# cornell-c2s2/dsp

Measured on AMD Instinct MI355X. Metric: MFCC frames/sec (512-pt FFT, 40 mel, 13 coeffs), higher is better.
Workload: dtype f32

## Files before the change

dsp_amd/csrc/mfcc_device.hpp:

```cpp
#pragma once

#include <hip/hip_runtime.h>

#include <type_traits>

#include "mfcc_kernels.hpp"

namespace dsp {

namespace {

struct c32 { float x, y; };
typedef float f2v __attribute__((ext_vector_type(2)));
typedef int i2v __attribute__((ext_vector_type(2)));
typedef float f4v __attribute__((ext_vector_type(4)));

__device__ __forceinline__ c32 cadd(c32 a, c32 b) { return {a.x + b.x, a.y + b.y}; }
__device__ __forceinline__ c32 csub(c32 a, c32 b) { return {a.x - b.x, a.y - b.y}; }
__device__ __forceinline__ c32 cmul(c32 a, c32 w) { return {a.x * w.x - a.y * w.y, a.x * w.y + a.y * w.x}; }
__device__ __forceinline__ c32 cmul_mi(c32 a) { return {a.y, -a.x}; }

__device__ __forceinline__ void radix4(c32 (&s)[4])
{
    const c32 t0 = cadd(s[0], s[2]), t1 = csub(s[0], s[2]);
    const c32 t2 = cadd(s[1], s[3]), t3 = cmul_mi(csub(s[1], s[3]));
    s[0] = cadd(t0, t2);
    s[1] = cadd(t1, t3);
    s[2] = csub(t0, t2);
    s[3] = csub(t1, t3);
}

__device__ __forceinline__ void wave_lds_sync()
{
    __builtin_amdgcn_fence(__ATOMIC_RELEASE, "wavefront");
    __builtin_amdgcn_wave_barrier();
    __builtin_amdgcn_fence(__ATOMIC_ACQUIRE, "wavefront");
}

__device__ __forceinline__ void swap_hi32(float &a, float &b)
{
    auto r = __builtin_amdgcn_permlane32_swap(__float_as_uint(a), __float_as_uint(b), false, false);
    a = __uint_as_float(r[0]);
    b = __uint_as_float(r[1]);
}
__device__ __forceinline__ void swap_odd16(float &a, float &b)
{
    auto r = __builtin_amdgcn_permlane16_swap(__float_as_uint(a), __float_as_uint(b), false, false);
    a = __uint_as_float(r[0]);
    b = __uint_as_float(r[1]);
}

template <int CTRL>
__device__ __forceinline__ float dpp(float v)
{
    return __int_as_float(__builtin_amdgcn_update_dpp(0, __float_as_int(v), CTRL, 0xF, 0xF, true));
}
constexpr int DPP_QUAD_1032 = 0xB1;
constexpr int DPP_QUAD_2301 = 0x4E;
constexpr int DPP_ROW_HALF_MIRROR = 0x141;
constexpr int DPP_ROW_MIRROR = 0x140;

template <int CTRL>
__device__ __forceinline__ unsigned dppu(unsigned v)
{
    return (unsigned)__builtin_amdgcn_update_dpp(0, (int)v, CTRL, 0xF, 0xF, true);
}
__device__ __forceinline__ float wave_max_nonneg(float f)
{
    unsigned v = __float_as_uint(f);
    v = max(v, dppu<DPP_QUAD_1032>(v));
    v = max(v, dppu<DPP_QUAD_2301>(v));
    v = max(v, dppu<DPP_ROW_HALF_MIRROR>(v));
    v = max(v, dppu<DPP_ROW_MIRROR>(v));
    const unsigned r0 = __builtin_amdgcn_readlane(v, 0), r1 = __builtin_amdgcn_readlane(v, 16);
    const unsigned r2 = __builtin_amdgcn_readlane(v, 32), r3 = __builtin_amdgcn_readlane(v, 48);
    return __uint_as_float(max(max(r0, r1), max(r2, r3)));
}

constexpr int LDS_XCHG = 0;
constexpr int LDS_PART = 2048 + 64;
constexpr int LDS_LOGMEL = LDS_PART + 320;
constexpr int LDS_WAVE_BYTES = LDS_LOGMEL + 320;
constexpr int LDS_TILE_BYTES = 64 * 16 * 4;
constexpr int LDS_POOL_BYTES = 32 * 16;
constexpr int LDS_STOP_BYTES = 64 * kStopFusedUnits * 8;
static_assert(LDS_WAVE_BYTES % 16 == 0, "keep the carve 16-byte aligned");
struct FrameCursor {
    long f, chunk_end, chunk_first, stride, n;
    long clip;
    long jump_clips;
    int t, t0, fpc, chunk, jump_t;
    long clip0;
    __device__ __forceinline__ void init(long wave, long n_waves, int chunk_, long n_, int fpc_)
    {
        chunk = chunk_; n = n_; fpc = fpc_;
        stride = n_waves * chunk;
        chunk_first = wave * chunk;
        f = chunk_first;
        chunk_end = f + chunk < n ? f + chunk : n;
        clip0 = 0; t0 = 0; jump_clips = 0; jump_t = 0;
        if (fpc > 0) {
            clip0 = f / fpc; t0 = (int)(f - clip0 * fpc);
            jump_clips = stride / fpc; jump_t = (int)(stride - jump_clips * fpc);
        }
        clip = clip0; t = t0;
    }
    __device__ __forceinline__ bool valid() const { return f < n; }
    __device__ __forceinline__ void next(int step)
    {
        f += step;
        if (f >= chunk_end) {
            chunk_first += stride;
            f = chunk_first;
            chunk_end = f + chunk < n ? f + chunk : n;
            clip0 += jump_clips; t0 += jump_t;
            if (t0 >= fpc) { t0 -= fpc; ++clip0; }
            clip = clip0; t = t0;
        } else if (fpc > 0) {
            t += step;
            while (t >= fpc) { t -= fpc; ++clip; }
        }
    }
};

template <bool CLIPS>
struct WaveCursor {
    long f, off;
    long clip;
    long chunk_f, chunk_off;
    long chunk_clip;
    long stride_f, stride_off;
    long clip_off, clip_stride;
    long jump_clips;
    int remaining;
    int left, chunk;
    int t, t0, fpc, jump_t, hop;
    __device__ __forceinline__ void init(long wave, long n_waves, int chunk_, long n, int fpc_, int hop_, long clip_stride_)
    {
        chunk = chunk_; fpc = fpc_; hop = hop_; clip_stride = clip_stride_;
        stride_f = n_waves * chunk;
        chunk_f = wave * chunk;
        f = chunk_f;
        left = chunk - 1;
        const long n_chunks = (n + chunk - 1) / chunk;
        const long mine = wave < n_chunks ? (n_chunks - 1 - wave) / n_waves + 1 : 0;
        const bool owns_last = mine > 0 && (n_chunks - 1 - wave) % n_waves == 0;
        remaining = (int)(mine * chunk - (owns_last ? n_chunks * chunk - n : 0));
        clip = chunk_clip = 0; t = t0 = 0; jump_t = 0; jump_clips = 0; clip_off = 0;
        if (CLIPS) {
            chunk_clip = f / fpc; t0 = (int)(f - chunk_clip * fpc);
            jump_clips = stride_f / fpc; jump_t = (int)(stride_f - jump_clips * fpc);
            stride_off = jump_clips * clip_stride;
            chunk_off = chunk_clip * clip_stride;
            clip = chunk_clip; t = t0; clip_off = chunk_off;
            off = clip_off + (long)t * hop;
        } else {
            stride_off = stride_f * hop;
            chunk_off = chunk_f * hop;
            off = chunk_off;
        }
    }
    __device__ __forceinline__ bool valid() const { return remaining > 0; }
    __device__ __forceinline__ void next()
    {
        --remaining;
        const bool in_chunk = left > 0;
        left = in_chunk ? left - 1 : chunk - 1;
        chunk_f += in_chunk ? 0 : stride_f;
        f = in_chunk ? f + 1 : chunk_f;
        if (CLIPS) {
            const bool wrap = t + 1 == fpc;
            const int t_in = wrap ? 0 : t + 1;
            const long clip_in = clip + (wrap ? 1 : 0);
            const long clip_off_in = clip_off + (wrap ? clip_stride : 0);
            const long off_in = wrap ? clip_off_in : off + hop;
            const int t0_raw = t0 + (in_chunk ? 0 : jump_t);
            const bool carry = t0_raw >= fpc;
            t0 = carry ? t0_raw - fpc : t0_raw;
            chunk_clip += in_chunk ? 0 : jump_clips + (carry ? 1 : 0);
            chunk_off += in_chunk ? 0 : stride_off + (carry ? clip_stride : 0);
            t = in_chunk ? t_in : t0;
            clip = in_chunk ? clip_in : chunk_clip;
            clip_off = in_chunk ? clip_off_in : chunk_off;
            off = in_chunk ? off_in : chunk_off + t0 * hop;
        } else {
            chunk_off += in_chunk ? 0 : stride_off;
            off = in_chunk ? off + hop : chunk_off;
        }
    }
};

struct RaggedCursor {
    long f, off, clip;
    const ClipSpan *spans;
    const int *chunk_span;
    int chunk_k, n_waves;
    int remaining;
    int left, chunk;
    int t, clip_left;
    int hop, n_samples;
    __device__ __forceinline__ void enter(const ClipSpan &s)
    {
        t = (int)(f - s.frame0);
        off = s.off + (long)t * hop;
        clip_left = s.frames - 1 - t;
        n_samples = s.n;
    }
    __device__ __forceinline__ void init(long wave, long n_waves_, int chunk_, long n, int hop_, const ClipSpan *spans_, long n_spans)
    {
        chunk = chunk_; hop = hop_; n_waves = (int)n_waves_; spans = spans_;
        chunk_span = reinterpret_cast<const int *>(spans_ + n_spans);
        chunk_k = (int)wave;
        left = chunk - 1;
        const long n_chunks = (n + chunk - 1) / chunk;
        const long mine = wave < n_chunks ? (n_chunks - 1 - wave) / n_waves_ + 1 : 0;
        const bool owns_last = mine > 0 && (n_chunks - 1 - wave) % n_waves_ == 0;
        remaining = (int)(mine * chunk - (owns_last ? n_chunks * chunk - n : 0));
        f = (long)chunk_k * chunk; off = 0; clip = 0; t = 0; clip_left = 0; n_samples = 0;
        if (remaining > 0) { clip = chunk_span[chunk_k]; enter(spans[clip]); }
    }
    __device__ __forceinline__ bool valid() const { return remaining > 0; }
    __device__ __forceinline__ void next()
    {
        if (--remaining <= 0) return;
        if (left > 0 && clip_left > 0) {
            --left; ++f; --clip_left; ++t; off += hop;
            return;
        }
        if (left > 0) { --left; ++f; ++clip; }
        else {
            left = chunk - 1;
            chunk_k += n_waves;
            f = (long)chunk_k * chunk;
            clip = chunk_span[chunk_k];
        }
        enter(spans[clip]);
    }
};

struct ClipCursor {
    long f, off, clip;
    long n_clips, n_waves, clip_stride;
    const ClipSpan *spans;
    int left, remaining, t, hop, fpc, n_samples;
    __device__ __forceinline__ void enter()
    {
        t = 0;
        if (clip >= n_clips) { remaining = 0; return; }
        remaining = 2;
        if (spans) {
            const ClipSpan s = spans[clip];
            off = s.off; n_samples = s.n; left = s.frames - 1;
        } else {
            off = clip * clip_stride; left = fpc - 1;
        }
    }
    __device__ __forceinline__ void init(long wave, long n_waves_, long n_clips_, int fpc_, int hop_, long clip_stride_, const ClipSpan *spans_,
                                         int samples_per_clip)
    {
        n_clips = n_clips_; n_waves = n_waves_; clip_stride = clip_stride_; spans = spans_; hop = hop_; fpc = fpc_; n_samples = samples_per_clip;
        f = 0; off = 0; left = 0; clip = wave;
        enter();
    }
    __device__ __forceinline__ bool valid() const { return remaining > 0; }
    __device__ __forceinline__ void next()
    {
        ++f;
        if (left > 0) { --left; ++t; off += hop; }
        else { clip += n_waves; enter(); }
    }
};

__device__ __forceinline__ const Mfcc512Args *kernarg_of_mfcc512()
{
#if defined(__HIP_DEVICE_COMPILE__)
    return (const Mfcc512Args *)__builtin_amdgcn_kernarg_segment_ptr();
#else
    return nullptr;
#endif
}

}

}
```

dsp_amd/csrc/mfcc_kernels.hip:

```cpp
#include "diag_guard.hpp"
#include <hip/hip_runtime.h>

#include <algorithm>

#include "mfcc_device.hpp"

#ifndef DSP_DIAG_MODE
#define DSP_DIAG_MODE 0
#endif
#ifndef DSP_PREFETCH
#define DSP_PREFETCH 2
#endif
#ifndef DSP_PRIO_LOAD
#define DSP_PRIO_LOAD 0
#endif
#ifndef DSP_PRIO_FFT
#define DSP_PRIO_FFT 0
#endif
#ifndef DSP_PRIO_FFT2
#define DSP_PRIO_FFT2 1
#endif
#ifndef DSP_PRIO_UNT
#define DSP_PRIO_UNT 2
#endif
#ifndef DSP_PRIO_MEL
#define DSP_PRIO_MEL 3
#endif
#ifndef DSP_PRIO_TILE
#define DSP_PRIO_TILE 3
#endif
#define DSP_SETPRIO(from, to) do { if ((from) != (to)) __builtin_amdgcn_s_setprio(to); } while (0)

namespace dsp {

#ifdef DSP_PF_STAMPS
__device__ unsigned long long g_pf_stamps[8 * 1024];
#define PF_STAMP(k) do { if ((threadIdx.x & 63) == 0 && blockIdx.x < 256) g_pf_stamps[(blockIdx.x * 4 + (threadIdx.x >> 6)) * 8 + (k)] = __builtin_amdgcn_s_memtime(); } while (0)
hipError_t read_pf_stamps(unsigned long long *host, int count) { return hipMemcpyFromSymbol(host, HIP_SYMBOL(g_pf_stamps), sizeof(unsigned long long) * (size_t)count); }
#else
#define PF_STAMP(k) do { } while (0)
#endif

namespace {

template <typename V>
__device__ __forceinline__ V ld_frame(const V *p, bool stream) { return stream ? __builtin_nontemporal_load(p) : *p; }

template <int FLEN, int IN, bool STREAM>
__device__ __forceinline__ void load_frame(const void *__restrict__ base, long off, int lane, int frame_len, c32 (&z)[4])
{
#pragma unroll
    for (int a = 0; a < 4; ++a) {
        const int i = 2 * (lane + 64 * a);
        const int flen = FLEN ? FLEN : frame_len;
        const bool both = i + 1 < flen, one = i < flen;
        if (IN == 0) {
            const float *src = static_cast<const float *>(base) + off;
            if (both) {
                const f2v v = ld_frame(reinterpret_cast<const f2v *>(src + i), STREAM);
                z[a] = {v.x, v.y};
            } else if (one) {
                z[a] = {src[i], 0.0f};
            } else {
                z[a] = {0.0f, 0.0f};
            }
        } else if (IN == 1) {
            const short *src = static_cast<const short *>(base) + off;
            int v = 0;
            if (both) v = ld_frame(reinterpret_cast<const int *>(src + i), STREAM);
            else if (one) v = (int)(unsigned short)src[i];
            z[a] = {__int_as_float(v), 0.0f};
        } else {
            const short *src = static_cast<const short *>(base) + 2 * off;
            i2v v = {0, 0};
            if (both) v = ld_frame(reinterpret_cast<const i2v *>(src + 2 * i), STREAM);
            else if (one) v.x = *reinterpret_cast<const int *>(src + 2 * i);
            z[a] = {__int_as_float(v.x), __int_as_float(v.y)};
        }
    }
}

template <int IN>
__device__ __forceinline__ c32 unpack_pcm16(c32 raw)
{
    const int a = __float_as_int(raw.x), b = __float_as_int(raw.y);
    if (IN == 1) return {(float)(short)(a & 0xFFFF), (float)(a >> 16)};
    if (IN == 2) return {(float)(short)(a & 0xFFFF), (float)(short)(b & 0xFFFF)};
    return {(float)((short)(a & 0xFFFF) + (a >> 16)), (float)((short)(b & 0xFFFF) + (b >> 16))};
}

}

template <int DCT_SPLIT, int DCT_LEN, int GATHER, int FLEN, int IN, int TILE, bool CLIPS, int POOL = 0, bool RAGGED = false>
#ifndef DSP_WAVES_PER_EU
#define DSP_WAVES_PER_EU 4
#endif
__global__ __launch_bounds__(256) __attribute__((amdgpu_waves_per_eu(DSP_WAVES_PER_EU))) void mfcc512_wave_kernel(const Mfcc512Args args)
{
    static_assert(!POOL || (TILE && CLIPS), "pooling lives in the tile epilogue of the clip-mode kernel");
    static_assert(!RAGGED || (CLIPS && !POOL), "ragged batches: clip mode, coefficients stored");
    constexpr int KS = DCT_SPLIT == 2 ? DCT_LEN / 2 : DCT_LEN;
    constexpr int CT = DCT_SPLIT == 2 ? 2 : 1;
    constexpr int WAVE_BYTES = LDS_WAVE_BYTES + (TILE ? LDS_TILE_BYTES : 0) + (POOL == 1 ? LDS_POOL_BYTES : (POOL == 2 ? LDS_STOP_BYTES : 0));
    extern __shared__ __attribute__((aligned(16))) char smem[];
    const int lane = threadIdx.x & 63;
    const int wib = __builtin_amdgcn_readfirstlane(threadIdx.x >> 6);
    char *wl = smem + wib * WAVE_BYTES;
    float *etile = reinterpret_cast<float *>(wl + LDS_WAVE_BYTES);
    double *pool_acc = reinterpret_cast<double *>(wl + LDS_WAVE_BYTES + LDS_TILE_BYTES);
    (void)etile; (void)pool_acc;
    float2 *xchg = reinterpret_cast<float2 *>(wl + LDS_XCHG);
    float *pbuf = reinterpret_cast<float *>(wl + LDS_XCHG);
    float *part = reinterpret_cast<float *>(wl + LDS_PART);
    float *lmel = reinterpret_cast<float *>(wl + LDS_LOGMEL);

    const LaneTables512 *__restrict__ T = args.tables;

    float win[8];
    constexpr float in_scale = IN == 0 ? 1.0f : (IN == 3 ? 1.0f / 65536.0f : 1.0f / 32768.0f);
#pragma unroll
    for (int i = 0; i < 8; ++i) win[i] = T->win[i][lane] * in_scale;
    c32 tw1[3], tw2[3], tw3[3], twp[2];
#pragma unroll
    for (int q = 0; q < 3; ++q) {
        tw1[q] = {T->tw1[2 * q][lane], T->tw1[2 * q + 1][lane]};
        tw2[q] = {T->tw2[2 * q][lane], T->tw2[2 * q + 1][lane]};
        tw3[q] = {T->tw3[2 * q][lane], T->tw3[2 * q + 1][lane]};
    }
    twp[0] = {T->twp[0][lane], T->twp[1][lane]};
    twp[1] = {T->twp[2][lane], T->twp[3][lane]};
    float melw[kMelChunk];
#pragma unroll
    for (int i = 0; i < kMelChunk; ++i) melw[i] = T->mel_w[i][lane];
    const int mel_k0 = T->mel_k0[lane];
    int gat[GATHER];
#pragma unroll
    for (int g = 0; g < GATHER; ++g) gat[g] = T->mel_src[g][lane];
    float dctw[(DCT_LEN + 3) & ~3];
    constexpr bool A_IN_REGS = CT * KS <= 10 && !POOL;
    float dcta[CT][KS];
    float *a_lds = reinterpret_cast<float *>(smem + 4 * WAVE_BYTES);
    (void)a_lds;
    if (TILE && !A_IN_REGS) {
        for (int i = threadIdx.x; i < CT * KS * 64; i += 256) a_lds[i] = (&T->dct_a[0][0][0])[(i / (KS * 64)) * (kDctSteps * 64) + i % (KS * 64)];
        __syncthreads();
    }
    if (TILE && A_IN_REGS) {
#pragma unroll
        for (int ct = 0; ct < CT; ++ct)
#pragma unroll
            for (int s = 0; s < KS; ++s) dcta[ct][s] = T->dct_a[ct][s][lane];
    } else if (!TILE) {
#pragma unroll
        for (int i = 0; i < DCT_LEN; ++i) dctw[i] = T->dct_w[i][lane];
    }
    const int n_mels = args.n_mels, n_mfcc = args.n_mfcc;
    constexpr int DCT_STRIDE = (DCT_LEN + 3) & ~3;
    const int dct_rd = (lane % DCT_SPLIT) * DCT_STRIDE;
    const int lmel_wr = (lane / DCT_LEN) * DCT_STRIDE + lane % DCT_LEN;
    const int dct_c = lane / DCT_SPLIT;
    const bool dct_store = (lane % DCT_SPLIT == 0) && dct_c < n_mfcc;

    const int d0 = lane & 3, d1 = (lane >> 2) & 3, d2 = lane >> 4;
    const int w3base = 64 * d2 + 4 * (d0 ^ d2) + d1;
    const int r3base = 64 * d0 + 16 * d2 + d1;
    const int kap = T->kappa[lane];
    const int partner = T->partner[lane] << 2;
    const bool self_paired = kap == 0;

    if (lane == 0) part[kZeroSlot] = 0.0f;
    if (lane < 16) lmel[64 + lane] = 0.0f;
    lmel[lane] = 0.0f;
    wave_lds_sync();

    const long wave = (long)blockIdx.x * 4 + wib;
    const long n_waves = (long)gridDim.x * 4;
    const unsigned amin_u = __float_as_uint(args.amin);
    const float neg_top_db = -args.top_db;
    const int frame_len = args.frame_len;
    const long n_frames = args.n_frames;

    constexpr int PF = POOL == 1 ? 1 : DSP_PREFETCH;
    std::conditional_t<POOL != 0, ClipCursor, std::conditional_t<RAGGED, RaggedCursor, WaveCursor<CLIPS>>> pre;
    if constexpr (POOL != 0) pre.init(wave, n_waves, args.n_clips, args.frames_per_clip, args.hop, args.clip_stride, args.spans, args.samples_per_clip);
    else if constexpr (RAGGED) pre.init(wave, n_waves, args.chunk, n_frames, args.hop, args.spans, args.n_clips);
    else pre.init(wave, n_waves, args.chunk, n_frames, args.frames_per_clip, CLIPS ? args.hop : frame_len, args.clip_stride);
    c32 ring[PF][4] = {};
    long fq[PF], cq[PF];
    bool lastq[PF];
    long safe_off = 0;
    auto refill = [&](int d) {
        const bool live = pre.valid();
        if (live) safe_off = pre.off;
        load_frame<FLEN, IN, !CLIPS>(args.in, safe_off, lane, frame_len, ring[d]);
        fq[d] = live ? pre.f : -1; cq[d] = live ? pre.clip : 0; lastq[d] = live && (pre.left == 0 || pre.remaining == 1);
        if (live) pre.next();
    };
#pragma unroll
    for (int d = 0; d < PF; ++d) refill(d);
    if (POOL == 0 && fq[0] < 0) return;

    int pool_t = 0;
    if (POOL == 1 && lane < 32) { pool_acc[2 * lane] = 0.0; pool_acc[2 * lane + 1] = 0.0; }
    float *stop_small = reinterpret_cast<float *>(smem + 4 * WAVE_BYTES) + (TILE && !A_IN_REGS ? CT * KS * 64 : 0);
    (void)stop_small;
    float *svm_small = stop_small;
    (void)svm_small;
    if (POOL == 1) {
        const SvmModelDev &m = args.pool.svm;
        for (int i = threadIdx.x; i < m.n_features; i += 256) { svm_small[i] = m.offset[i]; svm_small[m.n_features + i] = m.scale[i]; }
        for (int i = threadIdx.x; i < m.n_sv; i += 256) svm_small[2 * m.n_features + i] = m.coef[i];
        __syncthreads();
    }
    if (POOL == 2) {
#pragma unroll
        for (int j = 0; j < kStopFusedUnits; ++j) pool_acc[kStopFusedUnits * lane + j] = 0.0;
        const StopModelDev &m = args.stop.m;
        int n_in = m.units[0], off = 0;
        for (int l = 1; l < 4; ++l) {
            const int n_w = n_in * m.units[l];
            for (int i = threadIdx.x; i < n_w; i += 256) stop_small[off + i] = m.kernel[l][i];
            for (int i = threadIdx.x; i < m.units[l]; i += 256) stop_small[off + n_w + i] = m.bias[l][i];
            off += n_w + m.units[l];
            n_in = m.units[l];
        }
        __syncthreads();
    }
    if (POOL != 0 && fq[0] < 0) return;
    auto pool_tile = [&](const f4v (&d)[CT], int count) {
        int lane = threadIdx.x & 63;
        asm volatile("" : "+v"(lane));
        const int n = lane & 15, q = lane >> 4;
#pragma unroll
        for (int ct = 0; ct < CT; ++ct)
#pragma unroll
            for (int j = 0; j < 4; ++j) etile[(16 * ct + 4 * q + j) * 16 + n] = d[ct][j];
        wave_lds_sync();
#ifdef DSP_DIAG_NO_POOL
        if (count < 0)
#endif
        if (lane < n_mfcc) {
#pragma clang fp contract(off)
            double pool_s = pool_acc[2 * lane], pool_q = pool_acc[2 * lane + 1];
            for (int t = 0; t < count; ++t) {
                const double v = (double)etile[lane * 16 + t];
                pool_s = pool_s + v;
                pool_q = pool_q + v * v;
            }
            pool_acc[2 * lane] = pool_s; pool_acc[2 * lane + 1] = pool_q;
        }
        pool_t += count;
        wave_lds_sync();
    };
    auto pool_finish = [&](long clip) {
#pragma clang fp contract(off)
        const Mfcc512Args *ap = kernarg_of_mfcc512();
        asm volatile("" : "+s"(ap));
        if (ap->spans) clip = ap->spans[clip].orig;
        const PoolSvmArgs &pool = ap->pool;
        const SvmModelDev &m = pool.svm;
        PF_STAMP(0);
        float *z = etile;
        int lane = threadIdx.x & 63;
        asm volatile("" : "+v"(lane));
        if (lane < n_mfcc) {
            const double pool_s = pool_acc[2 * lane], pool_q = pool_acc[2 * lane + 1];
            pool_acc[2 * lane] = 0.0; pool_acc[2 * lane + 1] = 0.0;
            const double mean = pool_s / (double)pool_t;
            const double var = pool_q / (double)pool_t - mean * mean;
            const float f_mean = (float)mean, f_std = sqrtf((float)(var > 0 ? var : 0));
            const float *off_l = svm_small, *scl_l = svm_small + m.n_features;
            z[lane] = (f_mean - off_l[lane]) * scl_l[lane];
            z[n_mfcc + lane] = (f_std - off_l[n_mfcc + lane]) * scl_l[n_mfcc + lane];
            if (pool.feat) {
                pool.feat[clip * 2L * n_mfcc + lane] = f_mean;
                pool.feat[clip * 2L * n_mfcc + n_mfcc + lane] = f_std;
            }
        }
        wave_lds_sync();
        PF_STAMP(1);
        float term = 0.0f;
#ifdef DSP_DIAG_NO_SVM
        if (m.n_sv < 0)
#endif
        for (int sidx = lane; sidx < m.n_sv; sidx += 64) {
            const float *sv = m.sv + (long)sidx * m.n_features;
            float d2 = 0.0f;
            int j = 0;
            for (; j + 8 <= m.n_features; j += 8) {
                float v[8];
#pragma unroll
                for (int k = 0; k < 8; ++k) v[k] = sv[j + k];
#pragma unroll
                for (int k = 0; k < 8; ++k) {
                    const float dd = z[j + k] - v[k];
                    d2 = d2 + dd * dd;
                }
            }
            for (; j < m.n_features; ++j) {
                const float dd = z[j] - sv[j];
                d2 = d2 + dd * dd;
            }
            term = term + svm_small[2 * m.n_features + sidx] * expf(-m.gamma * d2);
        }
        PF_STAMP(2);
        for (int o = 32; o > 0; o >>= 1) term += __shfl_xor(term, o);
        PF_STAMP(3);
        if (lane == 0) {
            const float score = term + m.rho;
            int label;
            float p1;
#ifdef DSP_DIAG_NO_SVMTAIL
            label = score > 0; p1 = score;
#else
            svm_binary_tail(score, m.prob_a, m.prob_b, label, p1);
#endif
            pool.labels[clip] = label;
            if (pool.decision) pool.decision[clip] = score;
            if (pool.prob1) pool.prob1[clip] = p1;
        }
        PF_STAMP(4);
        wave_lds_sync();
        PF_STAMP(5);
        pool_t = 0;
    };
    auto stop_tile = [&](const f4v (&d)[CT], int count) {
        const Mfcc512Args *ap = kernarg_of_mfcc512();
        asm volatile("" : "+s"(ap));
        const StopModelDev &m = ap->stop.m;
        int lane = threadIdx.x & 63;
        asm volatile("" : "+v"(lane));
        const int n = lane & 15, q = lane >> 4;
#pragma unroll
        for (int j = 0; j < 4; ++j) etile[(4 * q + j) * 16 + n] = d[0][j];
        wave_lds_sync();
        const int c = lane & 15, tq = lane >> 4;
        const bool live_c = c < m.n_coef;
        const f4v *A = reinterpret_cast<const f4v *>(m.fold_a);
        double acc[kStopFusedUnits];
#pragma unroll
        for (int j = 0; j < kStopFusedUnits; ++j) acc[j] = pool_acc[kStopFusedUnits * lane + j];
#pragma unroll 1
        for (int k0 = 0; k0 < 4; k0 += 2) {
            f4v a[2];
            float x[2];
#pragma unroll
            for (int k = 0; k < 2; ++k) {
                const int tt = 4 * tq + k0 + k, t = pool_t + tt;
                const bool on = live_c && tt < count && t < m.max_frames;
                a[k] = A[on ? c * m.max_frames + t : 0];
                x[k] = on ? etile[c * 16 + tt] : 0.0f;
            }
#pragma unroll
            for (int k = 0; k < 2; ++k) {
                const double xd = (double)x[k];
#pragma unroll
                for (int j = 0; j < kStopFusedUnits; ++j) acc[j] = fma((double)a[k][j], xd, acc[j]);
            }
        }
#pragma unroll
        for (int j = 0; j < kStopFusedUnits; ++j) pool_acc[kStopFusedUnits * lane + j] = acc[j];
        pool_t += count;
        wave_lds_sync();
    };
    auto stop_finish = [&](long clip) {
#pragma clang fp contract(off)
        const Mfcc512Args *ap = kernarg_of_mfcc512();
        asm volatile("" : "+s"(ap));
        if (ap->spans) clip = ap->spans[clip].orig;
        const StopModelDev &m = ap->stop.m;
        int lane = threadIdx.x & 63;
        asm volatile("" : "+v"(lane));
        double acc[kStopFusedUnits];
#pragma unroll
        for (int j = 0; j < kStopFusedUnits; ++j) {
            acc[j] = pool_acc[kStopFusedUnits * lane + j];
            pool_acc[kStopFusedUnits * lane + j] = 0.0;
            for (int o = 32; o > 0; o >>= 1) acc[j] += __shfl_xor(acc[j], o);
        }
        if (lane == 0) {
            const int u1 = m.units[0];
            const int Tc = pool_t < m.max_frames ? pool_t : m.max_frames;
            float *h = etile;
#pragma unroll
            for (int j = 0; j < kStopFusedUnits; ++j)
                if (j < u1) {
                    const float sum = (float)((double)m.bias[0][j] + m.pad_b[(long)Tc * u1 + j] + acc[j]);
                    h[j] = sum > 0.0f ? sum : 0.0f;
                }
            int n_in = u1, off = 0;
            for (int l = 1; l < 4; ++l) {
                const int n_out = m.units[l];
                const float *src = h + ((l - 1) & 1) * kStopMaxUnits;
                float *dst = h + (l & 1) * kStopMaxUnits;
                const float *wl_ = stop_small + off, *bl_ = wl_ + n_in * n_out;
                off += n_in * n_out + n_out;
                for (int j = 0; j < n_out; ++j) {
                    float sum = bl_[j];
                    for (int i = 0; i < n_in; ++i) sum = sum + wl_[i * n_out + j] * src[i];
                    dst[j] = (l < 3 && !(sum > 0.0f)) ? 0.0f : sum;
                }
                n_in = n_out;
            }
            ap->stop.prob[clip] = 1.0f / (1.0f + expf(-h[kStopMaxUnits]));
        }
        pool_t = 0;
        wave_lds_sync();
    };
    (void)pool_tile; (void)pool_finish; (void)pool_t; (void)stop_tile; (void)stop_finish;

    int slot = 0;
    long fb0 = 0, fb1 = 0;
    auto flush = [&](int count) {
        wave_lds_sync();
        int lane = threadIdx.x & 63;
        if (POOL) asm volatile("" : "+v"(lane));
        const int n = lane & 15, q = lane >> 4;
        float ev[KS];
        unsigned mx = amin_u;
        if (A_IN_REGS) {
#pragma unroll
            for (int s = 0; s < KS; ++s) ev[s] = etile[64 * s + 16 * q + (n ^ s)];
#pragma unroll
            for (int s = 0; s < KS; ++s) mx = max(mx, __float_as_uint(ev[s]));
        } else {
#pragma unroll 2
            for (int s = 0; s < KS; ++s) mx = max(mx, __float_as_uint(etile[64 * s + 16 * q + (n ^ s)]));
        }
        {
            auto r = __builtin_amdgcn_permlane16_swap(mx, mx, false, false);
            mx = max(r[0], r[1]);
            r = __builtin_amdgcn_permlane32_swap(mx, mx, false, false);
            mx = max(r[0], r[1]);
        }
        const float rinv = __builtin_amdgcn_rcpf(__uint_as_float(mx));
        const float k10 = 3.01029995663981195f;
        f4v acc[CT][2];
#pragma unroll
        for (int ct = 0; ct < CT; ++ct) acc[ct][0] = acc[ct][1] = f4v{0.0f, 0.0f, 0.0f, 0.0f};
        auto kstep = [&](int s, float e_s, int par) {
            const float ec = __uint_as_float(max(__float_as_uint(e_s), amin_u));
            float db = k10 * __builtin_amdgcn_logf(ec * rinv);
            db = __builtin_amdgcn_fmed3f(db, neg_top_db, 0.0f);
            if (4 * s + q >= n_mels) db = 0.0f;
#pragma unroll
            for (int ct = 0; ct < CT; ++ct) {
                const float a = A_IN_REGS ? dcta[ct][s < KS ? s : 0] : a_lds[(ct * KS + s) * 64 + lane];
                acc[ct][par] = __builtin_amdgcn_mfma_f32_16x16x4f32(a, db, acc[ct][par], 0, 0, 0);
            }
        };
        if (A_IN_REGS) {
#pragma unroll
            for (int s = 0; s < KS; ++s) kstep(s, ev[s], s & 1);
        } else {
            static_assert(KS % 2 == 0, "two accumulator chains");
#pragma unroll 1
            for (int s = 0; s < KS; s += 2) {
                kstep(s, etile[64 * s + 16 * q + (n ^ s)], 0);
                kstep(s + 1, etile[64 * (s + 1) + 16 * q + (n ^ (s + 1))], 1);
            }
        }
        if (POOL) {
            f4v dd[CT];
#pragma unroll
            for (int ct = 0; ct < CT; ++ct) dd[ct] = acc[ct][0] + acc[ct][1];
            wave_lds_sync();
#ifdef DSP_DIAG_NO_POOLTILE
            if (dd[0][0] == 123.456f) args.pool.labels[0] = 1;
            return;
#endif
            if (POOL == 2) { if constexpr (CT == 1) stop_tile(dd, count); }
            else pool_tile(dd, count);
            return;
        }
        const long fl = (n < 8 ? fb0 : fb1 - 8) + n;
        const bool ok = n < count && fl < n_frames;
#pragma unroll
        for (int ct = 0; ct < CT; ++ct) {
            const f4v d = acc[ct][0] + acc[ct][1];
#pragma unroll
            for (int j = 0; j < 4; ++j) {
                const int c = 16 * ct + 4 * q + j;
                if (ok && c < n_mfcc) args.out[fl * n_mfcc + c] = d[j];
            }
        }
        wave_lds_sync();
    };
    (void)flush;

    auto step = [&](int rd) -> bool {
        c32 (&nxt)[4] = ring[rd];
        const long f = fq[rd];
        const long clip_f = cq[rd];
        const bool last_f = lastq[rd];
        (void)clip_f; (void)last_f;
        c32 s[4];
        DSP_SETPRIO(DSP_PRIO_TILE, DSP_PRIO_LOAD);
#pragma unroll
        for (int a = 0; a < 4; ++a) {
            const c32 x = IN == 0 ? nxt[a] : unpack_pcm16<IN>(nxt[a]);
            s[a] = {x.x * win[2 * a], x.y * win[2 * a + 1]};
        }
#if !(DSP_DIAG_MODE & 2)
        refill(rd);
#else
        fq[rd] = pre.valid() ? pre.f : -1; if (pre.valid()) pre.next();
#endif
        const bool more = fq[(rd + 1) % PF] >= 0;
#if DSP_DIAG_MODE == 1
        {
            float c = ((s[0].x + s[0].y) + (s[1].x + s[1].y)) + ((s[2].x + s[2].y) + (s[3].x + s[3].y));
            c += dpp<DPP_QUAD_1032>(c);
            if (dct_store) args.out[f * n_mfcc + dct_c] = c;
        }
        return more;
#endif

        DSP_SETPRIO(DSP_PRIO_LOAD, DSP_PRIO_FFT);
        radix4(s);
#pragma unroll
        for (int q = 1; q < 4; ++q) s[q] = cmul(s[q], tw1[q - 1]);
        swap_hi32(s[0].x, s[2].x); swap_hi32(s[0].y, s[2].y);
        swap_hi32(s[1].x, s[3].x); swap_hi32(s[1].y, s[3].y);
        swap_odd16(s[0].x, s[1].x); swap_odd16(s[0].y, s[1].y);
        swap_odd16(s[2].x, s[3].x); swap_odd16(s[2].y, s[3].y);
        radix4(s);
#pragma unroll
        for (int q = 1; q < 4; ++q) s[q] = cmul(s[q], tw2[q - 1]);
#pragma unroll
        for (int p = 0; p < 4; ++p) xchg[(lane ^ (4 * p)) + 64 * p] = {s[p].x, s[p].y};
        wave_lds_sync();
#pragma unroll
        for (int c = 0; c < 4; ++c) {
            const float2 v = xchg[64 * d1 + 16 * d2 + 4 * (c ^ d1) + d0];
            s[c] = {v.x, v.y};
        }
        wave_lds_sync();
        DSP_SETPRIO(DSP_PRIO_FFT, DSP_PRIO_FFT2);
#ifdef DSP_DIAG_SNOPS
#pragma unroll
        for (int i_ = 0; i_ < DSP_DIAG_SNOPS; ++i_) asm volatile("s_nop 0");
#endif
#ifdef DSP_DIAG_VNOPS
#pragma unroll
        for (int i_ = 0; i_ < DSP_DIAG_VNOPS; ++i_) asm volatile("v_mov_b32 %0, %0" : "+v"(s[i_ & 3].x));
#endif
        radix4(s);
#pragma unroll
        for (int q = 1; q < 4; ++q) s[q] = cmul(s[q], tw3[q - 1]);
#pragma unroll
        for (int o = 0; o < 4; ++o) xchg[w3base + 16 * o] = {s[o].x, s[o].y};
        wave_lds_sync();
#pragma unroll
        for (int dd = 0; dd < 4; ++dd) {
            const float2 v = xchg[r3base + 4 * (dd ^ d0)];
            s[dd] = {v.x, v.y};
        }
        wave_lds_sync();

        DSP_SETPRIO(DSP_PRIO_FFT2, DSP_PRIO_UNT);
        radix4(s);
        c32 b, d;
        b.x = __int_as_float(__builtin_amdgcn_ds_bpermute(partner, __float_as_int(s[3].x)));
        b.y = __int_as_float(__builtin_amdgcn_ds_bpermute(partner, __float_as_int(s[3].y)));
        d.x = __int_as_float(__builtin_amdgcn_ds_bpermute(partner, __float_as_int(s[2].x)));
        d.y = __int_as_float(__builtin_amdgcn_ds_bpermute(partner, __float_as_int(s[2].y)));
        b.x = self_paired ? s[0].x : b.x; b.y = self_paired ? s[0].y : b.y;
        d.x = self_paired ? s[3].x : d.x; d.y = self_paired ? s[3].y : d.y;
        float P[4];
#pragma unroll
        for (int h = 0; h < 2; ++h) {
            const c32 x = s[h], v = h == 0 ? b : d;
            const c32 E = {x.x + v.x, x.y - v.y};
            const c32 O = {x.x - v.x, x.y + v.y};
            const c32 Tw = cmul(O, twp[h]);
            const float xr = E.x + Tw.y, xi = E.y - Tw.x;
            const float mr = E.x - Tw.y, mi = E.y + Tw.x;
            P[2 * h] = xr * xr + xi * xi;
            P[2 * h + 1] = mr * mr + mi * mi;
        }
        const float p128 = 4.0f * (s[2].x * s[2].x + s[2].y * s[2].y);
        pbuf[kap] = P[0];
        pbuf[64 + kap] = P[2];
        pbuf[192 - kap] = P[3];
        pbuf[256 - kap] = P[1];
        if (self_paired) pbuf[128] = p128;
        DSP_SETPRIO(DSP_PRIO_UNT, DSP_PRIO_MEL);
        wave_lds_sync();

        {
            const float *rd = pbuf + mel_k0;
            float acc = 0.0f;
#pragma unroll
            for (int i = 0; i < kMelChunk; ++i) acc = fmaf(melw[i], rd[i], acc);
            part[lane] = acc;
        }
        wave_lds_sync();
        float e = part[gat[0]];
#pragma unroll
        for (int g = 1; g < GATHER; ++g) e += part[gat[g]];
        if (lane >= n_mels) e = 0.0f;

        DSP_SETPRIO(DSP_PRIO_MEL, DSP_PRIO_TILE);
        if (TILE) {
            if ((slot & 7) == 0) { if (slot == 0) fb0 = f; else fb1 = f; }
            etile[16 * lane + (slot ^ (lane >> 2))] = e;
            const bool clip_ends = POOL && last_f;
            if (clip_ends) PF_STAMP(6);
            if (++slot == 16 || !more || clip_ends) { flush(slot); slot = 0; }
#if !defined(DSP_DIAG_NO_POOLTILE) && !defined(DSP_DIAG_NO_POOLFINISH)
            if (clip_ends) { if (POOL == 2) stop_finish(clip_f); else pool_finish(clip_f); }
#endif
            return more;
        }

        const float k10 = 3.01029995663981195f;
        if (args.log_mode != 0) {
            const float top = __uint_as_float(max(__float_as_uint(wave_max_nonneg(e)), amin_u));
            const float top_db_val = k10 * __builtin_amdgcn_logf(top);
            if (args.frame_max != nullptr) {
                if (lane == 0) args.frame_max[f] = top_db_val;
                return more;
            }
            const float floor_db = args.clip_floor ? args.clip_floor[clip_f] : top_db_val + neg_top_db;
            const float ec = __uint_as_float(max(__float_as_uint(e), amin_u));
            const float db = fmaxf(k10 * __builtin_amdgcn_logf(ec), floor_db);
            if (lane < n_mels) lmel[lmel_wr] = db;
        } else {
            const float ref = __uint_as_float(max(__float_as_uint(wave_max_nonneg(e)), amin_u));
            const float ec = __uint_as_float(max(__float_as_uint(e), amin_u));
            float db = k10 * __builtin_amdgcn_logf(ec * __builtin_amdgcn_rcpf(ref));
            db = __builtin_amdgcn_fmed3f(db, neg_top_db, 0.0f);
            if (lane < n_mels) lmel[lmel_wr] = db;
        }
        wave_lds_sync();

        {
            const float *rd = lmel + dct_rd;
            float c = 0.0f;
#pragma unroll
            for (int i = 0; i + 4 <= DCT_LEN; i += 4) {
                const float4 v = *reinterpret_cast<const float4 *>(rd + i);
                c = fmaf(dctw[i], v.x, c);
                c = fmaf(dctw[i + 1], v.y, c);
                c = fmaf(dctw[i + 2], v.z, c);
                c = fmaf(dctw[i + 3], v.w, c);
            }
            if (DCT_LEN % 4) {
                const float2 v = *reinterpret_cast<const float2 *>(rd + (DCT_LEN & ~3));
                c = fmaf(dctw[DCT_LEN & ~3], v.x, c);
                c = fmaf(dctw[(DCT_LEN & ~3) + 1], v.y, c);
            }
            c += dpp<DPP_QUAD_1032>(c);
            if (DCT_SPLIT == 4) c += dpp<DPP_QUAD_2301>(c);
            if (dct_store) args.out[f * n_mfcc + dct_c] = c;
        }
        wave_lds_sync();
        return more;
    };

    static_assert(DSP_PREFETCH >= 1 && DSP_PREFETCH <= 3, "prefetch ring depth");
    while (true) {
        if (!step(0)) return;
        if (PF > 1 && !step(PF > 1 ? 1 : 0)) return;
        if (PF > 2 && !step(PF > 2 ? 2 : 0)) return;
    }
}


#define DSP_FOR_SHAPES(X) X(4, 10, 3) X(4, 10, 6) X(4, 16, 3) X(4, 16, 6) X(2, 20, 3) X(2, 20, 6)

template <int S, int L>
static size_t lds_bytes(bool tile, int pool = 0, int stop_small_floats = 0)
{
    constexpr int KS = S == 2 ? L / 2 : L, CT = S == 2 ? 2 : 1;
    return (size_t)4 * (LDS_WAVE_BYTES + (tile ? LDS_TILE_BYTES : 0) + (pool == 1 ? LDS_POOL_BYTES : (pool == 2 ? LDS_STOP_BYTES : 0))) +
           (tile && (CT * KS > 10 || pool) ? (size_t)CT * KS * 64 * 4 : 0) + (pool ? (size_t)((stop_small_floats + 3) & ~3) * 4 : 0);
}

static int stop_small_floats(const StopModelDev &m)
{
    int n = 0;
    for (int l = 1; l < 4; ++l) n += m.units[l - 1] * m.units[l] + m.units[l];
    return n;
}

template <int S, int L, int G>
constexpr bool kHas400 = (S == 4 && L == 10 && G == 3) || (S == 2 && L == 20 && G == 3);

template <int S, int L, int G>
static int flen_of(int frame_len) { return frame_len == 512 ? 512 : (frame_len == 400 && kHas400<S, L, G> ? 400 : 0); }

template <int S, int L, int G, int FLEN, int IN, int TILE>
static void launch_flen(const Mfcc512Args &args, bool clips, dim3 g, dim3 b, size_t lds, hipStream_t stream)
{
    if (args.spans) hipLaunchKernelGGL((mfcc512_wave_kernel<S, L, G, FLEN, IN, TILE, true, 0, true>), g, b, lds, stream, args);
    else if (IN == 0 && !clips) hipLaunchKernelGGL((mfcc512_wave_kernel<S, L, G, FLEN, 0, TILE, false>), g, b, lds, stream, args);
    else hipLaunchKernelGGL((mfcc512_wave_kernel<S, L, G, FLEN, IN, TILE, true>), g, b, lds, stream, args);
}

template <int S, int L, int G, int IN, int TILE>
static hipError_t launch_one(const Mfcc512Args &args, bool clips, int blocks, hipStream_t stream)
{
    const size_t lds = lds_bytes<S, L>(TILE);
    const dim3 g(blocks), b(256);
    const int flen = flen_of<S, L, G>(args.frame_len);
    if (flen == 512) launch_flen<S, L, G, 512, IN, TILE>(args, clips, g, b, lds, stream);
    else if (flen == 400) { if constexpr (kHas400<S, L, G>) launch_flen<S, L, G, 400, IN, TILE>(args, clips, g, b, lds, stream); }
    else launch_flen<S, L, G, 0, IN, TILE>(args, clips, g, b, lds, stream);
    return hipGetLastError();
}

hipError_t launch_mfcc512_pool(const Mfcc512Args &args, int dct_split, int dct_len, int gather, int blocks, hipStream_t stream)
{
    if (args.frames_per_clip <= 0 || args.chunk != args.frames_per_clip || args.log_mode != 0 || args.in_kind < 0 || args.in_kind > 3 || !args.pool.labels ||
        args.pool.svm.n_features != 2 * args.n_mfcc || args.pool.svm.n_features > 64 || args.pool.svm.n_sv < 1 || args.pool.svm.n_sv > kSvmFused512MaxSv)
        return hipErrorInvalidConfiguration;
    const dim3 g(blocks), b(256);
    if (args.in_kind != 0) {
#define DSP_LAUNCH_POOL_PCM(S, L, G)                                                                                        \
        if (dct_split == S && dct_len == L && gather == G && args.frame_len == 400) {                                        \
            const size_t lds = lds_bytes<S, L>(true, 1, 2 * args.pool.svm.n_features + args.pool.svm.n_sv);                 \
            if (args.in_kind == 1) hipLaunchKernelGGL((mfcc512_wave_kernel<S, L, G, 400, 1, 1, true, 1>), g, b, lds, stream, args);      \
            else if (args.in_kind == 2) hipLaunchKernelGGL((mfcc512_wave_kernel<S, L, G, 400, 2, 1, true, 1>), g, b, lds, stream, args); \
            else hipLaunchKernelGGL((mfcc512_wave_kernel<S, L, G, 400, 3, 1, true, 1>), g, b, lds, stream, args);          \
            return hipGetLastError();                                                                                       \
        }
        DSP_LAUNCH_POOL_PCM(4, 10, 3)
        DSP_LAUNCH_POOL_PCM(2, 20, 3)
#undef DSP_LAUNCH_POOL_PCM
        return hipErrorInvalidConfiguration;
    }
#define DSP_LAUNCH_POOL(S, L, G)                                                                                            \
    if (dct_split == S && dct_len == L && gather == G) {                                                                    \
        const size_t lds = lds_bytes<S, L>(true, 1, 2 * args.pool.svm.n_features + args.pool.svm.n_sv);                    \
        const int flen = flen_of<S, L, G>(args.frame_len);                                                                  \
        if (flen == 512) hipLaunchKernelGGL((mfcc512_wave_kernel<S, L, G, 512, 0, 1, true, 1>), g, b, lds, stream, args);   \
        else if (flen == 400) {                                                                                             \
            if constexpr (kHas400<S, L, G>) hipLaunchKernelGGL((mfcc512_wave_kernel<S, L, G, 400, 0, 1, true, 1>), g, b, lds, stream, args); \
        } else hipLaunchKernelGGL((mfcc512_wave_kernel<S, L, G, 0, 0, 1, true, 1>), g, b, lds, stream, args);             \
        return hipGetLastError();                                                                                           \
    }
    DSP_FOR_SHAPES(DSP_LAUNCH_POOL)
#undef DSP_LAUNCH_POOL
    return hipErrorInvalidConfiguration;
}

typedef void (*StopKernel)(const Mfcc512Args);
static StopKernel stop_kernel_of(int in_kind, int gather, int frame_len)
{
    if (in_kind == 1) return mfcc512_wave_kernel<4, 10, 3, 400, 1, 1, true, 2>;
    if (in_kind == 2) return mfcc512_wave_kernel<4, 10, 3, 400, 2, 1, true, 2>;
    if (in_kind == 3) return mfcc512_wave_kernel<4, 10, 3, 400, 3, 1, true, 2>;
    if (gather == 3 && frame_len == 400) return mfcc512_wave_kernel<4, 10, 3, 400, 0, 1, true, 2>;
    if (gather == 3) return mfcc512_wave_kernel<4, 10, 3, 0, 0, 1, true, 2>;
    if (gather == 6) return mfcc512_wave_kernel<4, 10, 6, 0, 0, 1, true, 2>;
    return nullptr;
}

int mfcc512_stop_grid(int blocks, const StopModelDev &m, int in_kind, int gather, int frame_len)
{
    const StopKernel kernel = stop_kernel_of(in_kind, gather, frame_len);
    if (!kernel) return blocks;
    const size_t lds = lds_bytes<4, 10>(true, 2, stop_small_floats(m));
    int per_cu = 0, dev = 0, n_cu = 0;
    if (hipOccupancyMaxActiveBlocksPerMultiprocessor(&per_cu, kernel, 256, lds) != hipSuccess || per_cu < 1) per_cu = 1;
    if (hipGetDevice(&dev) == hipSuccess && hipDeviceGetAttribute(&n_cu, hipDeviceAttributeMultiprocessorCount, dev) == hipSuccess && n_cu > 0)
        blocks = std::min(blocks, per_cu * n_cu);
    return std::max(blocks, 1);
}

hipError_t launch_mfcc512_stop(const Mfcc512Args &args, int dct_split, int dct_len, int gather, int blocks, hipStream_t stream)
{
    const StopModelDev &m = args.stop.m;
    if (args.frames_per_clip <= 0 || args.chunk != args.frames_per_clip || args.log_mode != 0 || args.in_kind < 0 || args.in_kind > 3 || !args.stop.prob ||
        (args.in_kind != 0 && !(gather == 3 && args.frame_len == 400)) || dct_split != 4 || dct_len != 10 || m.n_coef != args.n_mfcc || m.n_coef > 16 || m.units[0] < 1 || m.units[0] > kStopFusedUnits ||
        !m.fold_a || !m.pad_b)
        return hipErrorInvalidConfiguration;
    for (int l = 1; l < 4; ++l)
        if (m.units[l] < 1 || m.units[l] > kStopMaxUnits) return hipErrorInvalidConfiguration;
    const size_t lds = lds_bytes<4, 10>(true, 2, stop_small_floats(m));
    const StopKernel kernel = stop_kernel_of(args.in_kind, gather, args.frame_len);
    if (!kernel) return hipErrorInvalidConfiguration;
    blocks = mfcc512_stop_grid(blocks, m, args.in_kind, gather, args.frame_len);
    hipLaunchKernelGGL(kernel, dim3(blocks), dim3(256), lds, stream, args);
    return hipGetLastError();
}

hipError_t launch_mfcc512(const Mfcc512Args &args, int dct_split, int dct_len, int gather, int blocks,
                          hipStream_t stream, bool tile)
{
    const bool clips = args.frames_per_clip > 0 || args.spans;
    if (tile && (args.log_mode != 0 || args.chunk % 8 != 0)) return hipErrorInvalidConfiguration;
    if (args.spans && args.n_clips <= 0) return hipErrorInvalidConfiguration;
    if (args.in_kind != 0) {
        if (!(dct_split == 4 && dct_len == 10 && gather == 3) || !tile || !clips) return hipErrorInvalidConfiguration;
        if (args.in_kind == 1) return launch_one<4, 10, 3, 1, 1>(args, true, blocks, stream);
        if (args.in_kind == 2) return launch_one<4, 10, 3, 2, 1>(args, true, blocks, stream);
        if (args.in_kind == 3) return launch_one<4, 10, 3, 3, 1>(args, true, blocks, stream);
        return hipErrorInvalidConfiguration;
    }
#define DSP_LAUNCH(S, L, G)                                                                  \
    if (dct_split == S && dct_len == L && gather == G)                                       \
        return tile ? launch_one<S, L, G, 0, 1>(args, clips, blocks, stream)                 \
                    : launch_one<S, L, G, 0, 0>(args, clips, blocks, stream);
    DSP_FOR_SHAPES(DSP_LAUNCH)
#undef DSP_LAUNCH
    return hipErrorInvalidConfiguration;
}

__global__ void clip_floor_kernel(const float *__restrict__ frame_max, long n_clips, int fpc, float top_db,
                                  float *__restrict__ clip_floor)
{
    const long c = (long)blockIdx.x * blockDim.x + threadIdx.x;
    if (c >= n_clips) return;
    float m = -INFINITY;
    for (int t = 0; t < fpc; ++t) m = fmaxf(m, frame_max[c * fpc + t]);
    clip_floor[c] = m - top_db;
}

hipError_t launch_clip_floor(const float *frame_max, long n_clips, int frames_per_clip, float top_db, float *clip_floor,
                             hipStream_t stream)
{
    if (n_clips <= 0) return hipSuccess;
    hipLaunchKernelGGL(clip_floor_kernel, dim3((unsigned)((n_clips + 255) / 256)), dim3(256), 0, stream, frame_max, n_clips,
                       frames_per_clip, top_db, clip_floor);
    return hipGetLastError();
}

__global__ void clip_floor_ragged_kernel(const float *__restrict__ frame_max, const ClipSpan *__restrict__ spans, long n_spans, float top_db,
                                         float *__restrict__ clip_floor)
{
    const long c = (long)blockIdx.x * blockDim.x + threadIdx.x;
    if (c >= n_spans) return;
    const ClipSpan s = spans[c];
    float m = -INFINITY;
    for (int t = 0; t < s.frames; ++t) m = fmaxf(m, frame_max[s.frame0 + t]);
    clip_floor[c] = m - top_db;
}

hipError_t launch_clip_floor_ragged(const float *frame_max, const ClipSpan *spans, long n_spans, float top_db, float *clip_floor, hipStream_t stream)
{
    if (n_spans <= 0) return hipSuccess;
    hipLaunchKernelGGL(clip_floor_ragged_kernel, dim3((unsigned)((n_spans + 255) / 256)), dim3(256), 0, stream, frame_max, spans, n_spans,
                       top_db, clip_floor);
    return hipGetLastError();
}

__global__ void ragged_chunk_map_kernel(const ClipSpan *__restrict__ spans, long n_spans, int chunk, int *__restrict__ chunk_span)
{
    const long c = (long)blockIdx.x * blockDim.x + threadIdx.x;
    if (c >= n_spans) return;
    const ClipSpan s = spans[c];
    for (long k = (s.frame0 + chunk - 1) / chunk; k * chunk < s.frame0 + s.frames; ++k) chunk_span[k] = (int)c;
}

hipError_t launch_ragged_chunk_map(const ClipSpan *spans, long n_spans, int chunk, int *chunk_span, hipStream_t stream)
{
    if (n_spans <= 0) return hipSuccess;
    if (chunk <= 0) return hipErrorInvalidValue;
    hipLaunchKernelGGL(ragged_chunk_map_kernel, dim3((unsigned)((n_spans + 255) / 256)), dim3(256), 0, stream, spans, n_spans, chunk, chunk_span);
    return hipGetLastError();
}

int mfcc512_lds_bytes_per_block(bool tile) { return (int)lds_bytes<4, 10>(tile); }

template <int S, int L, int G, int TILE>
static int occupancy_one(bool full)
{
    int n = 0;
    const size_t lds = lds_bytes<S, L>(TILE);
    hipError_t e = full ? hipOccupancyMaxActiveBlocksPerMultiprocessor(&n, mfcc512_wave_kernel<S, L, G, 512, 0, TILE, false>, 256, lds)
                        : hipOccupancyMaxActiveBlocksPerMultiprocessor(&n, mfcc512_wave_kernel<S, L, G, 0, 0, TILE, false>, 256, lds);
    return e == hipSuccess && n > 0 ? n : 4;
}

int mfcc512_blocks_per_cu(int dct_split, int dct_len, int gather, bool full, bool tile)
{
#define DSP_OCC(S, L, G) \
    if (dct_split == S && dct_len == L && gather == G) return tile ? occupancy_one<S, L, G, 1>(full) : occupancy_one<S, L, G, 0>(full);
    DSP_FOR_SHAPES(DSP_OCC)
#undef DSP_OCC
    return 4;
}

}
```

Measured before the change: 2.394 billion.

## Fuse windowing into first radix-4 and defer prefetch refill past first stage

Multiplies the window directly into the first radix-4 butterfly with FMAs instead of in a separate pass. The prefetch refill for the next frame is moved behind a scheduling barrier after the first FFT stage, so the load issue overlaps FFT arithmetic rather than sitting ahead of it. The main loop is restructured to run full PF-deep rounds without per-step exit checks, followed by a drain tail. A full memory waitcnt is added after pool/stop finishing. The aim is fewer instructions and less branch overhead on the hot path, at the cost of more complex loop-exit logic and a possible extra stall from the drain.

```diff
diff --git a/dsp_amd/csrc/mfcc_device.hpp b/dsp_amd/csrc/mfcc_device.hpp
--- a/dsp_amd/csrc/mfcc_device.hpp
+++ b/dsp_amd/csrc/mfcc_device.hpp
@@ -35,6 +35,11 @@
     __builtin_amdgcn_fence(__ATOMIC_RELEASE, "wavefront");
     __builtin_amdgcn_wave_barrier();
     __builtin_amdgcn_fence(__ATOMIC_ACQUIRE, "wavefront");
+}
+
+__device__ __forceinline__ void mem_drain()
+{
+    __builtin_amdgcn_s_waitcnt(0);
 }
 
 __device__ __forceinline__ void swap_hi32(float &a, float &b)
diff --git a/dsp_amd/csrc/mfcc_kernels.hip b/dsp_amd/csrc/mfcc_kernels.hip
--- a/dsp_amd/csrc/mfcc_kernels.hip
+++ b/dsp_amd/csrc/mfcc_kernels.hip
@@ -496,18 +496,14 @@
         (void)clip_f; (void)last_f;
         c32 s[4];
         DSP_SETPRIO(DSP_PRIO_TILE, DSP_PRIO_LOAD);
-#pragma unroll
-        for (int a = 0; a < 4; ++a) {
-            const c32 x = IN == 0 ? nxt[a] : unpack_pcm16<IN>(nxt[a]);
-            s[a] = {x.x * win[2 * a], x.y * win[2 * a + 1]};
-        }
-#if !(DSP_DIAG_MODE & 2)
+        c32 xin[4];
+#pragma unroll
+        for (int a = 0; a < 4; ++a) xin[a] = IN == 0 ? nxt[a] : unpack_pcm16<IN>(nxt[a]);
+#if DSP_DIAG_MODE == 1
+#pragma unroll
+        for (int a = 0; a < 4; ++a) s[a] = {xin[a].x * win[2 * a], xin[a].y * win[2 * a + 1]};
         refill(rd);
-#else
-        fq[rd] = pre.valid() ? pre.f : -1; if (pre.valid()) pre.next();
-#endif
         const bool more = fq[(rd + 1) % PF] >= 0;
-#if DSP_DIAG_MODE == 1
         {
             float c = ((s[0].x + s[0].y) + (s[1].x + s[1].y)) + ((s[2].x + s[2].y) + (s[3].x + s[3].y));
             c += dpp<DPP_QUAD_1032>(c);
@@ -517,13 +513,30 @@
 #endif
 
         DSP_SETPRIO(DSP_PRIO_LOAD, DSP_PRIO_FFT);
-        radix4(s);
+        {
+            const float p2x = xin[2].x * win[4], p2y = xin[2].y * win[5], p3x = xin[3].x * win[6], p3y = xin[3].y * win[7];
+            const c32 t0 = {__builtin_fmaf(xin[0].x, win[0], p2x), __builtin_fmaf(xin[0].y, win[1], p2y)};
+            const c32 t1 = {__builtin_fmaf(xin[0].x, win[0], -p2x), __builtin_fmaf(xin[0].y, win[1], -p2y)};
+            const c32 t2 = {__builtin_fmaf(xin[1].x, win[2], p3x), __builtin_fmaf(xin[1].y, win[3], p3y)};
+            const c32 t3 = cmul_mi(c32{__builtin_fmaf(xin[1].x, win[2], -p3x), __builtin_fmaf(xin[1].y, win[3], -p3y)});
+            s[0] = cadd(t0, t2);
+            s[1] = cadd(t1, t3);
+            s[2] = csub(t0, t2);
+            s[3] = csub(t1, t3);
+        }
 #pragma unroll
         for (int q = 1; q < 4; ++q) s[q] = cmul(s[q], tw1[q - 1]);
         swap_hi32(s[0].x, s[2].x); swap_hi32(s[0].y, s[2].y);
         swap_hi32(s[1].x, s[3].x); swap_hi32(s[1].y, s[3].y);
         swap_odd16(s[0].x, s[1].x); swap_odd16(s[0].y, s[1].y);
         swap_odd16(s[2].x, s[3].x); swap_odd16(s[2].y, s[3].y);
+        __builtin_amdgcn_sched_barrier(0);
+#if !(DSP_DIAG_MODE & 2)
+        refill(rd);
+#else
+        fq[rd] = pre.valid() ? pre.f : -1; if (pre.valid()) pre.next();
+#endif
+        const bool more = fq[(rd + 1) % PF] >= 0;
         radix4(s);
 #pragma unroll
         for (int q = 1; q < 4; ++q) s[q] = cmul(s[q], tw2[q - 1]);
@@ -607,10 +620,13 @@
             etile[16 * lane + (slot ^ (lane >> 2))] = e;
             const bool clip_ends = POOL && last_f;
             if (clip_ends) PF_STAMP(6);
-            if (++slot == 16 || !more || clip_ends) { flush(slot); slot = 0; }
+            if (++slot == 16 || !more || clip_ends) {
+                flush(slot);
+                slot = 0;
 #if !defined(DSP_DIAG_NO_POOLTILE) && !defined(DSP_DIAG_NO_POOLFINISH)
-            if (clip_ends) { if (POOL == 2) stop_finish(clip_f); else pool_finish(clip_f); }
-#endif
+                if (clip_ends) { if (POOL == 2) stop_finish(clip_f); else pool_finish(clip_f); mem_drain(); }
+#endif
+            }
             return more;
         }
 
@@ -660,10 +676,22 @@
     };
 
     static_assert(DSP_PREFETCH >= 1 && DSP_PREFETCH <= 3, "prefetch ring depth");
-    while (true) {
-        if (!step(0)) return;
-        if (PF > 1 && !step(PF > 1 ? 1 : 0)) return;
-        if (PF > 2 && !step(PF > 2 ? 2 : 0)) return;
+    if constexpr (PF == 1) {
+        while (step(0)) { }
+    } else {
+        while (true) {
+            bool full = true;
+#pragma unroll
+            for (int d = 0; d < PF; ++d) full = full && fq[d] >= 0;
+            if (!full) break;
+#pragma unroll
+            for (int d = 0; d < PF; ++d) step(d);
+        }
+#pragma unroll
+        for (int d = 0; d + 1 < PF; ++d) {
+            if (fq[d] < 0) return;
+            step(d);
+        }
     }
 }
 
```

After: 2.389 billion. About the same (-0.2%).
